# arbobendik/web-ray-tracer

Measured on AMD Instinct MI355X. Metric: Mray/s at 1080p (spp x bounces x pixels / s), higher is better.
Workload: dtype f32

## Files before the change

web-ray-tracer_amd/csrc/flx_frame_common.h:

```cpp
#pragma once
#include "flx_kernels.h"
#include "flx_kernel_util.h"
#include "flx_wavefront_common.h"

namespace flx {

#ifndef FLX_WF_WALK_THREADS
#define FLX_WF_WALK_THREADS 1024
#endif
#ifndef FLX_WF_WAVES_PER_EU
#define FLX_WF_WAVES_PER_EU 4
#endif
#ifndef FLX_WF_LDS_TOTAL
#define FLX_WF_LDS_TOTAL (156 * 1024)
#endif
#ifndef FLX_WF_INNER
#define FLX_WF_INNER 8
#endif
#ifndef FLX_WF_UNROLL
#define FLX_WF_UNROLL 8
#endif
#ifndef FLX_WF_BATCH
#define FLX_WF_BATCH 24
#endif
#ifndef FLX_WF_DRAWS_PER_WAVE
#define FLX_WF_DRAWS_PER_WAVE 16
#endif
#ifndef FLX_FRAME_SHADERS_FRONT
#define FLX_FRAME_SHADERS_FRONT 3
#endif
#ifndef FLX_FRAME_PROLOGUE_WAVES
#define FLX_FRAME_PROLOGUE_WAVES 2
#endif
#ifndef FLX_FRAME_READY_UNITS
#define FLX_FRAME_READY_UNITS 32
#endif

typedef const __attribute__((address_space(4))) FrameArgs *FrameArgsP;
FLX_DEV const FrameArgs &frame_args(FrameArgsP p) { asm volatile("" : "+s"(p)); return *(const FrameArgs *)p; }
FLX_DEV FrameArgsP kernel_frame_args() { return (FrameArgsP)__builtin_amdgcn_kernarg_segment_ptr(); }
#define FLX_ARGS_OF(ab) const FrameArgs &A_ = frame_args(ab); const DeviceScene &sc = A_.sc; const DeviceFrame &fr = A_.fr; const WavefrontBuffers &wb = A_.wb; (void)sc; (void)fr; (void)wb

template <bool VER>
FLX_DEV uint32_t scene_version_of(const DeviceFrame &fr, uint32_t frameIdx) { return VER ? blockIdx.x * fr.frames + frameIdx : 0u; }

template <bool COUNT, bool LV = false, bool VER = false>
FLX_DEV bool shade0_tile(FrameArgsP ab, uint32_t tile, uint32_t lane, float4 h, WorkCounters &cnt, const FrameView *lv = nullptr) {
  uint32_t S, frameIdx, lightBase = 0;
  int tri;
  bool alive, compact;
  f3 camera;
  SurfaceCtx sf;
  float ndcX = 0.0f, ndcY = 0.0f;
  Hit hit;
  {
  FLX_ARGS_OF(ab);
  S = (uint32_t)fr.samples;
  uint32_t px, k;
  tile8_pixel(fr, tile, lane, px, k);
  const bool inFrame = px < fr.width && k < fr.rows;
  frameIdx = inFrame ? frame_index(fr, k) : 0u;
  camera = view_camera(view_at<LV>(fr, lv, frameIdx));
  tri = inFrame ? __float_as_int(h.w) : -1;
  alive = tri != -1 && fr.max_reflections > 0 && length(F3(1.0f, 1.0f, 1.0f) * F3(1.0f, 1.0f, 1.0f)) >= fr.min_importancy * SQRT3;
  hit.suv = F3(h.x, h.y, h.z); hit.triangleId = tri; hit.transformId = 0;
  compact = wb.rec0 != nullptr;
  if (alive) {
    hit.transformId = (int)sc.geometry[3 * tri + 2].y << 1;
    if (VER) { const uint32_t ver = scene_version_of<VER>(fr, frameIdx); hit.transformId += (int)(ver * 2u * sc.n_transforms); lightBase = ver * 6u * sc.n_lights; }
    const uint32_t py_gl = fr.height - 1u - image_row(fr, k);
    float viewDepthPerS;
    Ray pr;
    pr.origin = camera;
    pr.dir = primary_dir_v(fr, view_at<LV>(fr, lv, frameIdx), px, py_gl, ndcX, ndcY, viewDepthPerS);
    const WorkCounters before = cnt;
    shadeSurface<COUNT>(sc, fr, hit, pr, camera, sf, cnt);
    if (COUNT) {
      cnt.shades = before.shades + (cnt.shades - before.shades) * S;
      cnt.atlas_texels = before.atlas_texels + (cnt.atlas_texels - before.atlas_texels) * S;
    }
  }
  }
  for (uint32_t s = 0; s < S; s++) {
    FLX_ARGS_OF(ab);
    const uint32_t pathId = ((tile * S + s) << 6) | lane;
    float4 *rec = wb.rec + (size_t)pathId * 8;
    if (!alive) {
      if (tri != -1) finalize_path<LV>(fr, wb, pathId, F3(0.0f, 0.0f, 0.0f), F3(1.0f, 1.0f, 1.0f), F3(1.0f, 1.0f, 1.0f), lv);
      if (compact) wb.rec0[(size_t)pathId * 3] = make_float4(0.f, 0.f, 0.f, __int_as_float(RF_DEAD));
      else rec[0] = make_float4(0.f, 0.f, 0.f, __int_as_float(RF_DEAD));
      continue;
    }
    PathState p;
    PixelState ps;
    ps.firstRayLength = 1.0f; ps.glassFilter = 0.0f; ps.originalRMEx = 0.0f; ps.originalTPOx = 0.0f;
    ps.renderId.x = ps.renderId.y = ps.renderId.z = ps.renderId.w = 0.0f;
    ps.renderOriginalId = ps.renderId;
    ps.ndc_x = ndcX; ps.ndc_y = ndcY;
    ps.seed = view_at<LV>(fr, lv, frameIdx).random_seed;
    ps.lightBase = lightBase;
    ps.originalColor = F3(1.0f, 1.0f, 1.0f);
    p.hit = hit;
    p.lastHitPoint = camera;
    p.dontFilter = true;
    p.importancyFactor = F3(1.0f, 1.0f, 1.0f);
    const float cosSampleN = flx_cos((float)s);
    ShadeOut so;
    shadeSample(sc, fr, sf, ps, p, camera, cosSampleN, 0, so);
    const int flags = (p.dontFilter ? RF_DONT_FILTER : 0) | (so.needShadow ? RF_NEED_SHADOW : 0) | (so.shadowedNoWalk ? RF_SHADOWED_NO_WALK : 0) |
                      (nextBounceRuns(fr, 0, p.importancyFactor, ps.originalColor) ? 0 : RF_NO_CLOSEST);
    if (compact) {
      if (s == 0u) {
// ... 37 lines not shown
    const FrameView &v = view_at<LV>(fr, lv, frameIdx);
    pr.dir = primary_dir_v(fr, v, px, py_gl, nx, ny, viewDepthPerS);
    pr.origin = view_camera(v);
  }
  const uint32_t visitsBefore = cnt.primary_visits;
  const Hit hp = primaryWalkF(sc, inImage, pr, viewDepthPerS, cnt.primary_visits, xfBase);
  if (COUNT && wb.tileCost && wb.tileCostPrimary) {
    const uint32_t nTiles = ((fr.width + 7u) >> 3) * ((fr.rows + 7u) >> 3);
    atomicAdd(wb.tileCost + nTiles + tile, (unsigned long long)(cnt.primary_visits - visitsBefore));
  }
  float4 h = make_float4(hp.suv.x, hp.suv.y, hp.suv.z, __int_as_float(inImage ? hp.triangleId : -1));
  if (inImage) {
    if (COUNT && hp.triangleId != -1) cnt.primary_hits++;
    hits[(size_t)k * fr.width + px] = h;
  }
  return h;
}

template <bool COUNT, bool LV = false, bool VER = false>
FLX_DEV void shade_path(FrameArgsP ab, uint32_t pathId, WorkCounters &cnt, const FrameView *lv = nullptr) {
  FLX_ARGS_OF(ab);
  float4 *rec = wb.rec + (size_t)pathId * 8;
  uint32_t px, k, s;
  item_pixel(fr, pathId, px, k, s);
  const uint32_t frameIdx = frame_index(fr, k);
  const f3 camera = view_camera(view_at<LV>(fr, lv, frameIdx));
  PathState p;
  PixelState ps;
  ps.firstRayLength = 1.0f; ps.glassFilter = 0.0f; ps.originalRMEx = 0.0f; ps.originalTPOx = 0.0f;
  ps.renderId.x = ps.renderId.y = ps.renderId.z = ps.renderId.w = 0.0f;
  ps.renderOriginalId = ps.renderId;
  const float4 q0 = rec[0], q1 = rec[1], q2 = rec[2], q3 = rec[3], q6 = rec[6], q7 = rec[7];
  const int pb = __float_as_int(q3.w) + 1;
  p.ray.origin = F3(q0.x, q0.y, q0.z);
  p.lastHitPoint = p.ray.origin;
  p.ray.dir = F3(q1.x, q1.y, q1.z);
  p.hit.suv = F3(q2.x, q2.y, q2.z);
  p.hit.triangleId = __float_as_int(q2.w);
  p.hit.transformId = (int)sc.geometry[3 * p.hit.triangleId + 2].y << 1;
  if (VER) { const uint32_t ver = scene_version_of<VER>(fr, frameIdx); p.hit.transformId += (int)(ver * 2u * sc.n_transforms); ps.lightBase = ver * 6u * sc.n_lights; }
  p.dontFilter = (__float_as_int(q0.w) & RF_DONT_FILTER) != 0;
  p.importancyFactor = F3(q6.x, q6.y, q6.z);
  ps.originalColor = F3(q7.x, q7.y, q7.z);
  const uint32_t py_gl = fr.height - 1u - image_row(fr, k);
  float viewDepthPerS;
  (void)primary_dir_v(fr, view_at<LV>(fr, lv, frameIdx), px, py_gl, ps.ndc_x, ps.ndc_y, viewDepthPerS);
  ps.seed = view_at<LV>(fr, lv, frameIdx).random_seed;
  const float cosSampleN = flx_cos((float)s);
  ShadeOut so;
  bounceShade<COUNT>(sc, fr, ps, p, camera, cosSampleN, pb, so, cnt);
  const int flags = (p.dontFilter ? RF_DONT_FILTER : 0) | (so.needShadow ? RF_NEED_SHADOW : 0) | (so.shadowedNoWalk ? RF_SHADOWED_NO_WALK : 0) |
                    (nextBounceRuns(fr, pb, p.importancyFactor, ps.originalColor) ? 0 : RF_NO_CLOSEST);
  rec[0] = make_float4(p.ray.origin.x, p.ray.origin.y, p.ray.origin.z, __int_as_float(flags));
  rec[1] = make_float4(p.ray.dir.x, p.ray.dir.y, p.ray.dir.z, so.shadowLen);
  rec[2] = make_float4(so.shadowRay.origin.x, so.shadowRay.origin.y, so.shadowRay.origin.z, so.baseLuminance.x);
  rec[3] = make_float4(so.shadowRay.dir.x, so.shadowRay.dir.y, so.shadowRay.dir.z, __int_as_float(pb));
  rec[4] = make_float4(so.litColor.x, so.litColor.y, so.litColor.z, 0.0f);
  rec[6] = make_float4(p.importancyFactor.x, p.importancyFactor.y, p.importancyFactor.z, 0.0f);
  rec[7] = make_float4(ps.originalColor.x, ps.originalColor.y, ps.originalColor.z, 0.0f);
}

struct WalkLane {
  int st;
  uint32_t pathId; int flags; int pathBounce; float base;
  Ray nextRay, shadowRay; float shadowLen;
  WalkState w; WalkEntry cur;
  uint32_t v0;
};
FLX_DEV void walkLaneInit(WalkLane &L) {
  L.v0 = 0u;
  L.st = P_EMPTY; L.pathId = 0; L.flags = 0; L.pathBounce = 0; L.base = 0.0f;
  L.nextRay.origin = F3(0.f, 0.f, 0.f); L.nextRay.dir = L.nextRay.origin;
  L.shadowRay = L.nextRay; L.shadowLen = 0.0f;
  walkClearResults(L.w);
  L.w.src = L.nextRay; L.w.tR = L.nextRay; L.w.minLen = 0.0f; L.w.i = 0; L.w.cachedTI = 0;
  L.w.mode = 2;
  L.cur.e0 = L.cur.e1 = L.cur.e2 = make_float4(0.f, 0.f, 0.f, 0.f);
}
FLX_DEV const float4 *pix_part(const DeviceFrame &fr, const WavefrontBuffers &wb, uint32_t id) {
  uint32_t tile0, s0;
  item_tile(fr, id, tile0, s0);
  return wb.pix0 + (((size_t)tile0 << 6) | (id & 63u)) * 3;
}
#define FLX_WALK_LANE_FOLD(LV_, fr_, wb_, compactRecs_, L_, lv_, toShade_, ended_, costed_, stamp_)                              \
  do {                                                                                                                           \
    float4 *rec_ = (wb_).rec + (size_t)(L_).pathId * 8;                                                                          \
    const bool compact_ = (compactRecs_) && (L_).pathBounce == 0;                                                                \
    float4 q4_, q5_, q6_, q7_;                                                                                                   \
    const float4 *pp_ = nullptr;                                                                                                 \
    if (compact_) {                                                                                                              \
      pp_ = pix_part(fr_, wb_, (L_).pathId);                                                                                     \
      q4_ = (wb_).rec0[(size_t)(L_).pathId * 3 + 2]; q7_ = pp_[2];                                                               \
      q5_ = make_float4(0.0f, 0.0f, 0.0f, 0.0f); q6_ = make_float4(1.0f, 1.0f, 1.0f, 0.0f);                                      \
    } else {                                                                                                                     \
      q4_ = rec_[4]; q5_ = rec_[5]; q6_ = rec_[6]; q7_ = rec_[7];                                                                \
    }                                                                                                                            \
    const bool shadowed_ = ((L_).flags & RF_SHADOWED_NO_WALK) || (((L_).flags & RF_NEED_SHADOW) && (L_).w.shadowed);            \
    const f3 localColor_ = shadowed_ ? F3((L_).base, (L_).base, (L_).base) : F3(q4_.x, q4_.y, q4_.z);                            \
    const f3 importancy_ = F3(q6_.x, q6_.y, q6_.z), originalColor_ = F3(q7_.x, q7_.y, q7_.z);                                    \
    const f3 finalColor_ = F3(q5_.x, q5_.y, q5_.z) + localColor_ * importancy_;                                                  \
     \
    const float cost_ = (costed_) ? q5_.w + (float)(((stamp_) - ((uint32_t)(L_).flags >> 8)) & 0xffffffu) : 1.0f;      \
    bool cont_ = (L_).w.tri != -1;                                                                                               \
    if (cont_) cont_ = ((L_).pathBounce + 1) < (fr_).max_reflections && length(importancy_ * originalColor_) >= (fr_).min_importancy * SQRT3;      \
    if (cont_) {                                                                                                                 \
      if (compact_) {                                         \
        const float4 a_ = (wb_).rec0[(size_t)(L_).pathId * 3], bq_ = (wb_).rec0[(size_t)(L_).pathId * 3 + 1], p0_ = pp_[0];      \
        rec_[0] = make_float4(p0_.x, p0_.y, p0_.z, a_.w);                                                                        \
        rec_[1] = make_float4(a_.x, a_.y, a_.z, bq_.w);                                                                          \
        rec_[3] = make_float4(bq_.x, bq_.y, bq_.z, __int_as_float(0));                                                           \
        rec_[6] = make_float4(1.0f, 1.0f, 1.0f, 0.0f);                                                                           \
        rec_[7] = make_float4(q7_.x, q7_.y, q7_.z, 0.0f);                                                                        \
      }                                                                                                                          \
      rec_[5] = make_float4(finalColor_.x, finalColor_.y, finalColor_.z, (costed_) ? cost_ : 0.0f);                                                 \
      rec_[2] = make_float4((L_).w.suv.x, (L_).w.suv.y, (L_).w.suv.z, __int_as_float((L_).w.tri));                               \
      toShade_ = true;                                                                                                           \
    } else {                                                                                                                     \
      finalize_path<LV_>(fr_, wb_, (L_).pathId, finalColor_, importancy_, originalColor_, lv_, cost_);                           \
      ended_ = true;                                                                                                             \
    }                                                                                                                            \
    (L_).st = P_EMPTY;                                                                                                           \
  } while (0)

struct WalkRecord { float4 q0, q1, q2, q3; };
FLX_DEV void walkLaneFetchRecord(const DeviceFrame &fr, const WavefrontBuffers &wb, uint32_t id, bool compactFresh, WalkRecord &R) {
  const float4 *rec = wb.rec + (size_t)id * 8;
  if (compactFresh) {
    const float4 *pp = pix_part(fr, wb, id);
    const float4 a = wb.rec0[(size_t)id * 3], bq = wb.rec0[(size_t)id * 3 + 1];
    const float4 p0 = pp[0], p1 = pp[1], p2 = pp[2];
    R.q0 = make_float4(p0.x, p0.y, p0.z, a.w);
    R.q1 = make_float4(a.x, a.y, a.z, bq.w);
    R.q2 = make_float4(p1.x, p1.y, p1.z, p2.w);
    R.q3 = make_float4(bq.x, bq.y, bq.z, __int_as_float(0));
  } else {
    R.q0 = rec[0]; R.q1 = rec[1]; R.q2 = rec[2]; R.q3 = rec[3];
  }
}
template <bool COUNT>
FLX_DEV bool walkLaneInstall(uint32_t id, const WalkRecord &R, WalkLane &L, WorkCounters &cnt, uint32_t stamp = 0u ) {
  const int fl = __float_as_int(R.q0.w);
  if (fl & RF_DEAD) return true;
  L.pathId = id; L.flags = fl | (int)(stamp << 8); L.base = R.q2.w; L.pathBounce = __float_as_int(R.q3.w);
  L.nextRay.origin = F3(R.q0.x, R.q0.y, R.q0.z);
  L.nextRay.dir = F3(R.q1.x, R.q1.y, R.q1.z);
  L.shadowRay.origin = F3(R.q2.x, R.q2.y, R.q2.z);
  L.shadowRay.dir = F3(R.q3.x, R.q3.y, R.q3.z);
  L.shadowLen = R.q1.w;
  walkClearResults(L.w);
  L.w.mode = (fl & RF_NEED_SHADOW) ? 0 : 1;
  if (COUNT) { if (L.w.mode == 0) cnt.shadow_walks++; if (!(fl & RF_NO_CLOSEST)) cnt.closest_walks++; L.v0 = cnt.closest_visits + cnt.shadow_visits; }
  L.st = (L.w.mode == 1 && (fl & RF_NO_CLOSEST)) ? P_DONE : P_SETUP;
  return false;
}
template <bool COUNT>
FLX_DEV bool walkLaneLoad(const DeviceFrame &fr, const WavefrontBuffers &wb, uint32_t id, bool compactFresh, WalkLane &L, WorkCounters &cnt, uint32_t stamp = 0u) {
  WalkRecord R;
  walkLaneFetchRecord(fr, wb, id, compactFresh, R);
  return walkLaneInstall<COUNT>(id, R, L, cnt, stamp);
}
template <bool COUNT>
FLX_DEV void walkLaneSetup(const DeviceScene &sc, uint32_t nTransforms, const float4 *xf, float2 *myRays, const float4 *walkG, const float4 *ldsEntries, uint32_t ldsCount,
                           WalkLane &L, WorkCounters &cnt) {
  const bool shadowMode = L.w.mode == 0;
  const Ray src = shadowMode ? L.shadowRay : L.nextRay;
  walkSetupRays(sc, nTransforms, xf, myRays, src, shadowMode);
  L.w.tR = src; L.w.cachedTI = 0; L.w.minLen = shadowMode ? L.shadowLen : POW32; L.w.i = (int)sc.walk_root;
  reciprocalOfDir(sc, src.dir, src.origin, L.w.inv, L.w.fastDiv);
  L.st = P_WALKING;
  if (walkFetchG<COUNT>(walkG, ldsEntries, ldsCount, myRays, L.w, L.cur, cnt)) L.st = shadowMode ? P_SWITCH : P_DONE;
}
FLX_DEV void walkLaneSwitch(WalkLane &L) {
  if (L.st == P_SWITCH) {
    if (L.flags & RF_NO_CLOSEST) L.st = P_DONE;
    else { L.w.mode = 1; L.st = P_SETUP; }
  }
}
#ifndef FLX_WF_TRI_EARLY_FETCH
#define FLX_WF_TRI_EARLY_FETCH 1
#endif
#if FLX_WF_TRI_EARLY_FETCH && !(FLX_WF_LINK_KIND && FLX_WF_LINK_ISBOX)
#error "FLX_WF_TRI_EARLY_FETCH needs FLX_WF_LINK_KIND and FLX_WF_LINK_ISBOX: neither the arrival nor the trip's control may wait for the loaded entry"
#endif
FLX_DEV float4 walkAnyFloat4() {
  float x, y, z, w;
  asm volatile("" : "=v"(x)); asm volatile("" : "=v"(y)); asm volatile("" : "=v"(z)); asm volatile("" : "=v"(w));
  return make_float4(x, y, z, w);
}
#if FLX_WF_TRI_EARLY_FETCH
#define FLX_WALK_LANE_STEP(COUNT_, THICK_, walkG_, ldsEntries_, ldsCount_, myRays_, L_, cnt_)                                      \
  do {                                                                                                                           \
    WalkEntry nxt_;                                                                                                              \
    nxt_.e0 = walkAnyFloat4(); nxt_.e1 = walkAnyFloat4(); nxt_.e2 = walkAnyFloat4();                                             \
    if ((L_).st == P_WALKING) {                                                                                                  \
      bool ended_ = false;                                                                                                       \
      uint32_t here_ = (uint32_t)(L_).w.i;                                        \
      if (walkIsBoxL((L_).w)) walkBoxP<THICK_>((L_).w, (L_).cur); else (L_).w.i = __float_as_int((L_).cur.e2.y);                 \
      walkFetchIssue(walkG_, ldsEntries_, ldsCount_, (uint32_t)(L_).w.i, nxt_);                                                  \
      asm("" : "+v"(here_));                                                                                                     \
      if (linkKind(here_) != 1u) ended_ = walkTriT((L_).w, (L_).cur);                                                            \
      if (!ended_) ended_ = walkFetchArrive<COUNT_>(myRays_, (L_).w, nxt_, cnt_);                                                \
      if (ended_) (L_).st = ((L_).w.mode == 0) ? P_SWITCH : P_DONE;                                                              \
    }                                                                                                                            \
    (L_).cur = nxt_;                                                                                                             \
  } while (0)
// ... 68 lines not shown
```

web-ray-tracer_amd/csrc/flx_server.hip:

```cpp
#include <cstddef>
#include <cstdio>
#include <mutex>
#include "flx_server.h"
#include "flx_frame_common.h"

namespace flx {

#ifndef FLX_SERVER_RELAY_GROUPS
#define FLX_SERVER_RELAY_GROUPS 16
#endif
#ifndef FLX_SERVER_SHADERS
#define FLX_SERVER_SHADERS FLX_FRAME_SHADERS_FRONT
#endif
#ifndef FLX_SERVER_SHADERS_DEPTH2_MAX_TILES
#define FLX_SERVER_SHADERS_DEPTH2_MAX_TILES 24
#endif
#ifndef FLX_SERVER_SHADERS_DEPTH2
#define FLX_SERVER_SHADERS_DEPTH2 2
#endif
#ifndef FLX_SERVER_SHADE_PRIO
#define FLX_SERVER_SHADE_PRIO 0
#endif
#ifndef FLX_SERVER_PRIO
#define FLX_SERVER_PRIO 1
// ... 349 lines not shown
            if (fq_pop(ring(RK_WALK, slot), rctl(RK_WALK, slot), idle, nIdle, 1u, lane, id) != 0u) {
              if (mineIdle && id != WF_INVALID) newId = id;
              any = flx_ballot(mineIdle && id != WF_INVALID) != 0ull;
              got = true;
              break;
            }
            if (chunkNext == chunkEnd && fq_load(&rctl(RK_SHADE, slot)[2]) < FQ_LIMIT) {
              uint32_t unit = WF_INVALID;
              if (fq_pop(ring(RK_READY, slot), rctl(RK_READY, slot), 1ull, 1u, 1u, lane, unit) != 0u) {
                unit = __builtin_amdgcn_readfirstlane(unit);
                if (unit != WF_INVALID) { chunkNext = unit << 6; chunkEnd = chunkNext + 64u; }
                else if (lane == 0) { FLX_SERVER_ARGS(); atomicSub(&ctl[SC_ALIVE + slot], 64u); __hip_atomic_fetch_or(sa.error, WF_ERR_RING_SLOT, __ATOMIC_RELAXED, __HIP_MEMORY_SCOPE_SYSTEM); }
              }
            }
            if (chunkNext != chunkEnd && slotOf(chunkNext) == slot) {
              const uint32_t avail = chunkEnd - chunkNext;
              const uint32_t take = nIdle < avail ? nIdle : avail;
              if (mineIdle && rk < take) { newId = chunkNext + rk; newFresh = true; }
              chunkNext += take;
              got = true; any = true;
              break;
            }
          }
          if (!got || !any) break;
        }
        if (newId != WF_INVALID) { FLX_ARGS_OF(ab); walkLaneFetchRecord(fr, wb, newId, newFresh, newRec); }
      }
      if (flx_ballot(L.st == P_DONE) != 0ull) {
        FLX_ARGS_OF(ab);
        const bool compactRecs = wb.rec0 != nullptr;
        bool toShade = false, ended = false;
        const uint32_t slot = slotOf(L.pathId);
        if (L.st == P_DONE) FLX_WALK_LANE_FOLD(true, fr, wb, compactRecs, L, lv, toShade, ended, false, 0u);
        if (flx_ballot(ended) != 0ull) __builtin_amdgcn_fence(__ATOMIC_RELEASE, "workgroup");
        for (uint32_t s = 0; s < depth; s++) {
          fq_push(ring(RK_SHADE, s), rctl(RK_SHADE, s), toShade && slot == s, L.pathId, lane);
          const uint32_t e = (uint32_t)__popcll(flx_ballot(ended && slot == s));
          if (e != 0u && lane == 0) atomicSub(&ctl[SC_ALIVE + s], e);
        }
        worked();
      }
      {
        bool dead = false;
        if (newId != WF_INVALID) dead = walkLaneInstall<false>(newId, newRec, L, cnt);
        if (flx_ballot(dead) != 0ull) {
          const uint32_t dslot = slotOf(newId);
          for (uint32_t sl = 0; sl < depth; sl++) {
            const uint32_t nDead = (uint32_t)__popcll(flx_ballot(dead && dslot == sl));
            if (nDead != 0u && lane == 0) atomicSub(&ctl[SC_ALIVE + sl], nDead);
          }
        }
      }
      if (FLX_SERVER_PRIO) {
        const bool tail = fq_load(&ctl[SC_TILEDRY + P]) != 0u;
        if (tail && flx_ballot(L.st != P_EMPTY && slotOf(L.pathId) == P) != 0ull) __builtin_amdgcn_s_setprio(3); else __builtin_amdgcn_s_setprio(0);
      }
      walkLaneSwitch(L);
      if (flx_ballot(L.st == P_SETUP) != 0ull) {
        FLX_ARGS_OF(ab);
        if (L.st == P_SETUP) walkLaneSetup<false>(sc, nTransforms, VER ? ldsXf + (size_t)slotOf(L.pathId) * nTransforms * 4u : ldsXf, myRays, walkGV, ldsEntriesV, ldsCount, L, cnt);
      }
      if (flx_ballot(L.st == P_WALKING) == 0ull) {
        if (flx_ballot(L.st != P_EMPTY) != 0ull) continue;
        if (fq_load(&ctl[SC_EXIT]) != 0u) break;
        tryRotate();
        if (!mayRefill) __builtin_amdgcn_s_sleep(8);
        continue;
      }
    }
    {
#pragma unroll FLX_WF_UNROLL
      for (int it = 0; it < FLX_WF_INNER; it++) FLX_WALK_LANE_STEP(false, THICK, walkGV, ldsEntriesV, ldsCount, myRays, L, cnt);
    }
  }
  statAdd(SVS_WALK_TRIPS, statTrips); statAdd(SVS_WALK_LANE_TRIPS, statLaneTrips);
  leave();
}

bool server_kernel_fits(const DeviceScene &sc, uint32_t &ldsCount, uint32_t &ldsBytes, uint32_t xfSlots, uint32_t shadeWaves) {
  const uint32_t T = sc.n_transforms;
  if (shadeWaves == 0u) shadeWaves = (uint32_t)FLX_SERVER_SHADERS;
  const uint32_t walkThreads = FLX_WF_WALK_THREADS - 64u * shadeWaves;
  const uint32_t fixed = walkThreads * T * 40u + xfSlots * T * 64u + (SC_WORDS + SC_VIEW_WORDS) * 4u;
  if (fixed + 4096u > (uint32_t)FLX_WF_LDS_TOTAL) return false;
  ldsCount = ((uint32_t)FLX_WF_LDS_TOTAL - fixed) / 48u;
  if (ldsCount > sc.walk_hot) ldsCount = sc.walk_hot;
  ldsBytes = ldsCount * 48u + fixed;
  return true;
}

size_t server_rings_per_group() { return (size_t)SV_RINGS * FQ_SIZE; }

int launch_server(const DeviceScene &sc, const DeviceFrame &fr, const WavefrontBuffers &wb, const ServerArgs &sa, uint32_t compute_units, hipStream_t stream,
                  WalkLdsLaunch *ran) {
  uint32_t ldsCount = 0, ldsBytes = 0;
  const bool ver = sa.blobWords != 0u;
  if (sa.depth < 2u || sa.depth > SV_MAX_DEPTH) return -1;
  const uint32_t shadeWaves = sa.depth == 2u && sa.tilesPerSlot / compute_units <= (uint32_t)FLX_SERVER_SHADERS_DEPTH2_MAX_TILES ? (uint32_t)FLX_SERVER_SHADERS_DEPTH2 : (uint32_t)FLX_SERVER_SHADERS;
  if (!server_kernel_fits(sc, ldsCount, ldsBytes, ver ? sa.depth : 1u, shadeWaves)) return -1;
  if (ver && (sa.blobWords > SV_BLOB_WORDS || sa.blobWords != server_blob_words(sc.n_transforms, sc.n_lights))) return -1;
  static std::once_flag once[64];
  static bool ok[64];
  int dev = 0;
  if (hipGetDevice(&dev) != hipSuccess || dev < 0 || dev >= 64) return -1;
  static const void *const kernels[2][2] = { { (const void *)k_wf_server<false, false>, (const void *)k_wf_server<false, true> },
                                             { (const void *)k_wf_server<true, false>, (const void *)k_wf_server<true, true> } };
  std::call_once(once[dev], [&]() {
    ok[dev] = true;
    for (int k = 0; k < 4; k++) ok[dev] = hipFuncSetAttribute(kernels[k >> 1][k & 1], hipFuncAttributeMaxDynamicSharedMemorySize, 160 * 1024) == hipSuccess && ok[dev];
  });
  if (!ok[dev]) return -1;
  ServerKernelArgs ka;
  ka.fa.sc = sc; ka.fa.fr = fr; ka.fa.wb = wb; ka.sa = sa;
  const uint32_t tilesPerGroup = sa.tilesPerSlot / compute_units;
  uint32_t readyUnits = tilesPerGroup >= 48u ? (uint32_t)FLX_FRAME_READY_UNITS : tilesPerGroup / 2u;
  readyUnits = readyUnits < (uint32_t)FLX_FRAME_READY_UNITS / 4u ? (uint32_t)FLX_FRAME_READY_UNITS / 4u : (readyUnits > (uint32_t)FLX_FRAME_READY_UNITS ? (uint32_t)FLX_FRAME_READY_UNITS : readyUnits);
  uint32_t ldsCountArg = ldsCount, nTransformsArg = sc.n_transforms, shadeWavesArg = shadeWaves;
  void *args[] = { &ka, &ldsCountArg, &nTransformsArg, &shadeWavesArg, &readyUnits };
  (void)hipLaunchKernel(kernels[ver ? 1 : 0][sc.walk_thick_boxes != 0u ? 1 : 0], dim3(compute_units), dim3(FLX_WF_WALK_THREADS), args, ldsBytes, stream);
  if (ran) { ran->ldsCount = ldsCount; ran->pre = 1u; ran->kind = 4u; ran->nTransforms = sc.n_transforms; ran->boxTest = sc.walk_thick_boxes != 0u ? 1 : 0; }
  return 0;
}

}
```

web-ray-tracer_amd/csrc/flx_wavefront.hip:

```cpp
#include <atomic>
#include <mutex>
#include <cstdio>
#include "flx_kernels.h"
#include "flx_kernel_util.h"
#include "flx_wavefront_common.h"
#include "flx_frame_common.h"

namespace flx {


#ifndef FLX_WF_WALK_THREADS
#define FLX_WF_WALK_THREADS 1024
#endif
#ifndef FLX_WF_DRAWS_PER_WAVE
#define FLX_WF_DRAWS_PER_WAVE 16
#endif
#ifndef FLX_WF_PRETRANSFORM
#define FLX_WF_PRETRANSFORM 1
#endif
#ifndef FLX_WF_LDS_TOTAL
#define FLX_WF_LDS_TOTAL (156 * 1024)
#endif
#ifndef FLX_WF_INNER
#define FLX_WF_INNER 8
// ... 568 lines not shown
            }
          }
        }
        chunkNext += take;
      }
      if (COUNT) { const long long tl = clock64(); tLoad += tl - t1; }
      if (st == P_SWITCH) {
        if (flags & RF_NO_CLOSEST) st = P_DONE;
        else { w.mode = 1; st = P_SETUP; }
      }
      if (flx_ballot(st == P_SETUP) != 0ull) {
        if (st == P_SETUP) {
          const bool shadowMode = w.mode == 0;
          const Ray src = shadowMode ? shadowRay : nextRay;
          walkSetupRays(sc, nTransforms, ldsXf, myRays, src, shadowMode);
          w.tR = src; w.cachedTI = 0; w.minLen = shadowMode ? shadowLen : POW32; w.i = (int)sc.walk_root;
          reciprocalOfDir(sc, src.dir, src.origin, w.inv, w.fastDiv);
          st = P_WALKING;
          if (walkFetchP<COUNT>(sc, ldsEntries, ldsCount, myRays, w, cur, cnt)) st = shadowMode ? P_SWITCH : P_DONE;
        }
      }
      if (COUNT) tRefill += clock64() - t1;
      if (flx_ballot(st == P_WALKING) == 0ull) {
        if (itemsLeft || chunkNext != chunkEnd || flx_ballot(st == P_SWITCH || st == P_DONE) != 0ull) continue;
#if FLX_WF_CONSOLIDATE
        if (tailSynced) continue;
#endif
        break;
      }
    }
    long long t2 = COUNT ? clock64() : 0;
#pragma unroll FLX_WF_UNROLL
    for (int it = 0; it < FLX_WF_INNER; it++) {
      if (COUNT) diagIters++;
      if (st == P_WALKING) {
        bool ended = false;
        if (walkIsBoxT(cur)) walkBoxP(w, cur); else ended = walkTriT(w, cur);
        if (!ended) ended = walkFetchP<COUNT>(sc, ldsEntries, ldsCount, myRays, w, cur, cnt);
        if (ended) st = (w.mode == 0) ? P_SWITCH : P_DONE;
      }
#if FLX_DIAG_PAD_SALU
      { uint32_t a = 1, b = 2, c = 3, d = 4;
        for (int k = 0; k < FLX_DIAG_PAD_SALU / 4; k++) asm volatile("s_mov_b32 %0, %1\n s_mov_b32 %1, %2\n s_mov_b32 %2, %3\n s_mov_b32 %3, %0" : "+s"(a), "+s"(b), "+s"(c), "+s"(d) : : "scc"); }
#endif
#if FLX_DIAG_PAD_VALU
      { uint32_t a = lane, b = lane, c = lane, d = lane;
        for (int k = 0; k < FLX_DIAG_PAD_VALU / 4; k++) asm volatile("v_add_u32 %0, %0, 1\n v_add_u32 %1, %1, 1\n v_add_u32 %2, %2, 1\n v_add_u32 %3, %3, 1" : "+v"(a), "+v"(b), "+v"(c), "+v"(d)); }
#endif
    }
    if (COUNT) tInner += clock64() - t2;
  }
#if FLX_WF_CONSOLIDATE
  if (lane == 0) { atomicSub(&tailCtl[TC_LIVE], 1u); if (tailMode) { atomicSub(&tailCtl[TC_TAIL], 1u); atomicAnd(&tailCtl[TC_MASK], ~(1u << (threadIdx.x >> 6))); } }
#endif
  if (outValid) {
    for (uint32_t t = outUsed + lane; t < WF_OUT_CHUNK; t += 64u) listOut[outBase + t] = WF_INVALID;
  }
  if (COUNT && b == 0 && (cnt.closest_visits | cnt.shadow_visits) != 0u) atomicAdd(wb.counters + 23, (unsigned long long)cnt.closest_visits + cnt.shadow_visits);
  flush_counters<COUNT>(cnt, wb.counters);
  if (COUNT && lane == 0) {
    atomicAdd(wb.counters + 8 + 2 * (b < 4 ? b : 3), (unsigned long long)diagIters); atomicAdd(wb.counters + 9 + 2 * (b < 4 ? b : 3), (unsigned long long)diagBatches);
    const unsigned long long life = (unsigned long long)(clock64() - tStart);
    if (b == 0) {
      atomicAdd(wb.counters + 16, (unsigned long long)tFold); atomicAdd(wb.counters + 17, (unsigned long long)tRefill);
      atomicAdd(wb.counters + 18, (unsigned long long)tInner); atomicAdd(wb.counters + 19, life); atomicAdd(wb.counters + 20, 1ull);
      atomicAdd(wb.counters + 21, (unsigned long long)tLoad); atomicAdd(wb.counters + 22, (unsigned long long)tTail);
    }
    if (b < 4) {
      atomicAdd(wb.counters + 24 + 3 * b, life); atomicAdd(wb.counters + 25 + 3 * b, 1ull); atomicMax(wb.counters + 26 + 3 * b, life);
    }
  }
}

#ifndef FLX_FRAME_WALK_PRIO
#define FLX_FRAME_WALK_PRIO 0
#endif
#ifndef FLX_FRAME_SHADE_PRIO
#define FLX_FRAME_SHADE_PRIO 0
#endif
#ifndef FLX_FRAME_SHADERS
#define FLX_FRAME_SHADERS 2
#endif
#ifndef FLX_FRAME_SHADERS_FRONT
#define FLX_FRAME_SHADERS_FRONT 3
#endif
#ifndef FLX_FRAME_PROLOGUE_WAVES
#define FLX_FRAME_PROLOGUE_WAVES 2
#endif
#ifndef FLX_FRAME_GROUPS_PER_CU
#define FLX_FRAME_GROUPS_PER_CU 1
#endif
#ifndef FLX_FRAME_AUTO_MAX_ITEMS
#define FLX_FRAME_AUTO_MAX_ITEMS (64u << 20)
#endif
#ifndef FLX_FRAME_AUTO_MAX_ITEMS_FRONT
#define FLX_FRAME_AUTO_MAX_ITEMS_FRONT (128u << 20)
#endif
template <bool COUNT, bool FRONT, bool STAMP, bool THICK>
__device__ __forceinline__ void wf_frame_body(uint32_t total_items, uint32_t ldsCount, uint32_t nTransforms, uint32_t shadeWaves, uint32_t readyUnits) {
  const uint32_t n = total_items;
  if (n == 0u) return;
  const FrameArgsP argBase = kernel_frame_args();
#define FLX_FRAME_ARGS() FLX_ARGS_OF(argBase)
  const uint32_t WALK_WAVES = FLX_WF_WALK_THREADS / 64u - shadeWaves;
  uint32_t *frameRings; uint32_t samples; bool compactRecs;
  { FLX_FRAME_ARGS(); frameRings = wb.frameRings; samples = (uint32_t)fr.samples; compactRecs = wb.rec0 != nullptr; }
  extern __shared__ float4 ldsAll[];
  float4 *ldsEntries = ldsAll;
  float4 *ldsXf = ldsAll + (size_t)ldsCount * 3u;
  uint32_t *ctl = (uint32_t *)(ldsXf + (size_t)nTransforms * 4u);
  uint32_t *shadeRing = frameRings + (size_t)blockIdx.x * WF_FRAME_RINGS * FQ_SIZE, *walkRing = shadeRing + FQ_SIZE, *readyRing = walkRing + FQ_SIZE;
  constexpr bool front = FRONT;
  const uint32_t perTile = samples * 64u;
  float2 *raysBase = (float2 *)(ctl + FC_WORDS);
  {
    FLX_FRAME_ARGS();
    for (uint32_t t = threadIdx.x; t < ldsCount * 3u; t += FLX_WF_WALK_THREADS) ldsEntries[t] = sc.walk[t];
    for (uint32_t t = threadIdx.x; t < nTransforms * 4u; t += FLX_WF_WALK_THREADS) {
      const uint32_t tr = t >> 2, k = t & 3u, iI = 2u * tr + 1u;
      ldsXf[t] = k < 3u ? sc.rotation[3u * iI + k] : sc.shift[iI];
    }
  }
  if (threadIdx.x < (uint32_t)FC_WORDS) ctl[threadIdx.x] = 0u;
  __syncthreads();
  const uint32_t lane = threadIdx.x & 63u;
  const uint32_t wave = threadIdx.x >> 6;
  WorkCounters cnt = {};

  const uint32_t nTiles = n / perTile;
  auto makeTile = [&]() -> uint32_t {
    if (!FRONT) return 2u;
    FLX_FRAME_ARGS();
    uint32_t take = 0, tile = 0;
    if (lane == 0 && fq_load(&ctl[FC_RQ + 2]) < readyUnits) {
      const uint32_t before = atomicAdd(&ctl[FC_ALIVE], perTile);
      if (before + perTile > FQ_ALIVE_MAX) atomicSub(&ctl[FC_ALIVE], perTile);
      else { tile = atomicAdd(wb.walkQueue, 1u); take = 1; }
    }
    take = __builtin_amdgcn_readfirstlane(take);
    tile = __builtin_amdgcn_readfirstlane(tile);
    if (take == 0u) return 0u;
    if (tile >= nTiles) {
      if (lane == 0) atomicSub(&ctl[FC_ALIVE], perTile);
      return 2u;
    }
    if (wb.tileOrder) tile = __builtin_amdgcn_readfirstlane(wb.tileOrder[tile]);
    tile += wb.item_base / perTile;
    const float4 h = primary_tile<COUNT>(argBase, tile, lane, cnt);
    const bool runs = shade0_tile<COUNT>(argBase, tile, lane, h, cnt);
    if (flx_ballot(runs) == 0ull) {
      if (lane == 0) atomicSub(&ctl[FC_ALIVE], perTile);
    } else {
      for (uint32_t s0 = 0; s0 < samples; s0 += 64u)
        fq_push(readyRing, ctl + FC_RQ, s0 + lane < samples, tile * samples + s0 + lane, lane);
    }
    return 1u;
  };

  if (wave >= WALK_WAVES) {
    uint32_t idle = 0;
    bool frontDone = !front;
    uint32_t inject; { FLX_FRAME_ARGS(); inject = wb.inject; } asm volatile("" : "+s"(inject));
    if (FLX_FRAME_SHADE_PRIO) __builtin_amdgcn_s_setprio(FLX_FRAME_SHADE_PRIO);
    const long long tStartShade = COUNT ? clock64() : 0;
    uint32_t thinMarks = 0;
    for (;;) {
      FLX_FRAME_ARGS();
// ... 215 lines not shown
      }
      const long long tB2 = COUNT ? clock64() : 0; if (COUNT) tRefillT += tB2 - tB1;
      walkLaneSwitch(L);
      if (flx_ballot(L.st == P_SETUP) != 0ull) {
        FLX_FRAME_ARGS();
        if (L.st == P_SETUP) walkLaneSetup<COUNT>(sc, nTransforms, ldsXf, myRays, FLX_FETCH_G, FLX_FETCH_L, ldsCount, L, cnt);
      }
      if (COUNT) { const long long tB3 = clock64(); tSetupT += tB3 - tB2; tBlock += tB3 - tB0; }
      if (flx_ballot(L.st == P_WALKING) == 0ull) {
        if (flx_ballot(L.st != P_EMPTY) != 0ull) continue;
        if (front) {
          if (fq_load(&ctl[FC_DRY]) != 0u && chunkNext == chunkEnd && fq_load(&ctl[FC_ALIVE]) == 0u) break;
        } else if (!itemsLeft && chunkNext == chunkEnd && fq_load(&ctl[FC_ALIVE]) == 0u) break;
        if (fq_load(&ctl[FC_WQ + 2]) == 0u && (front ? (fq_load(&ctl[FC_RQ + 2]) == 0u || fq_load(&ctl[FC_SQ + 2]) >= FQ_LIMIT)
                                                     : !(itemsLeft && fq_load(&ctl[FC_SQ + 2]) < FQ_LIMIT && fq_load(&ctl[FC_ALIVE]) + 256u <= FQ_ALIVE_MAX))) {
          FLX_FRAME_ARGS();
          if (++idleSpins > (wb.watchdog ? wb.watchdog : FQ_WATCHDOG)) {
            if (lane == 0 && wb.error) __hip_atomic_fetch_or(wb.error, WF_ERR_WALK_WATCHDOG, __ATOMIC_RELAXED, __HIP_MEMORY_SCOPE_SYSTEM);
            if (COUNT && lane == 0) { for (uint32_t k = 0; k < 8u; k++) atomicMax(wb.counters + 50 + k, (unsigned long long)fq_load(&ctl[k]) + 1ull); atomicAdd(wb.counters + 58, 1ull); }
            break;
          }
          __builtin_amdgcn_s_sleep(8);
        }
        continue;
      }
    }
    const long long tT0 = COUNT ? clock64() : 0;
    {
#pragma unroll FLX_WF_UNROLL
      for (int it = 0; it < FLX_WF_INNER; it++) FLX_WALK_LANE_STEP(COUNT, THICK, FLX_FETCH_G, FLX_FETCH_L, ldsCount, myRays, L, cnt);
    }
    if (COUNT) tTrips += clock64() - tT0;
  }
  FLX_FRAME_ARGS();
  if (COUNT && (cnt.closest_visits | cnt.shadow_visits) != 0u) atomicAdd(wb.counters + 23, (unsigned long long)cnt.closest_visits + cnt.shadow_visits);
#if FLX_BOX_FALLBACK_COUNT
  if (COUNT && wave < WALK_WAVES) atomicAdd(wb.counters + 59, (unsigned long long)L.w.boxTests | (unsigned long long)L.w.boxExact << 32);
#endif
  if (COUNT && lane == 0) {
    const unsigned long long life = (unsigned long long)(clock64() - tStart);
    atomicAdd(wb.counters + 64, life); atomicMax(wb.counters + 65, life); atomicAdd(wb.counters + 66, 1ull);
    atomicAdd(wb.counters + 67, (unsigned long long)tBlock); atomicAdd(wb.counters + 68, (unsigned long long)tFoldT); atomicAdd(wb.counters + 69, (unsigned long long)tRefillT); atomicAdd(wb.counters + 70, (unsigned long long)tSetupT);
    atomicAdd(wb.counters + 71, (unsigned long long)tTrips); atomicAdd(wb.counters + 72, nBlocks); atomicAdd(wb.counters + 73, nOuter);
    atomicAdd(wb.counters + 74, (unsigned long long)tAcqT); atomicAdd(wb.counters + 75, (unsigned long long)tFoldOnlyT);
  }
  flush_counters<COUNT>(cnt, wb.counters);
#undef FLX_FETCH_G
#undef FLX_FETCH_L
#undef FLX_FRAME_ARGS
}
template <bool COUNT, bool FRONT>
__global__ __launch_bounds__(FLX_WF_WALK_THREADS, FLX_WF_WAVES_PER_EU) void k_wf_frame(FrameArgs , uint32_t total_items,
                                                                                    uint32_t ldsCount, uint32_t nTransforms, uint32_t shadeWaves, uint32_t readyUnits) {
  wf_frame_body<COUNT, FRONT, !FRONT, true>(total_items, ldsCount, nTransforms, shadeWaves, readyUnits);
}
template <bool COUNT, bool FRONT>
__global__ __launch_bounds__(FLX_WF_WALK_THREADS, FLX_WF_WAVES_PER_EU) void k_wf_frame_flat(FrameArgs , uint32_t total_items,
                                                                                         uint32_t ldsCount, uint32_t nTransforms, uint32_t shadeWaves, uint32_t readyUnits) {
  wf_frame_body<COUNT, FRONT, !FRONT, false>(total_items, ldsCount, nTransforms, shadeWaves, readyUnits);
}
template <bool COUNT>
__global__ __launch_bounds__(FLX_WF_WALK_THREADS, FLX_WF_WAVES_PER_EU) void k_wf_frame_stamped(FrameArgs , uint32_t total_items,
                                                                                            uint32_t ldsCount, uint32_t nTransforms, uint32_t shadeWaves, uint32_t readyUnits) {
  wf_frame_body<COUNT, true, true, true>(total_items, ldsCount, nTransforms, shadeWaves, readyUnits);
}
template <bool COUNT>
__global__ __launch_bounds__(FLX_WF_WALK_THREADS, FLX_WF_WAVES_PER_EU) void k_wf_frame_stamped_flat(FrameArgs , uint32_t total_items,
                                                                                                 uint32_t ldsCount, uint32_t nTransforms, uint32_t shadeWaves, uint32_t readyUnits) {
  wf_frame_body<COUNT, true, true, false>(total_items, ldsCount, nTransforms, shadeWaves, readyUnits);
}
static const void *frame_kernel(int which, bool count, bool thick) {
  static const void *const kernels[3][2][2] = {
    { { (const void *)k_wf_frame_flat<false, false>, (const void *)k_wf_frame<false, false> }, { (const void *)k_wf_frame_flat<true, false>, (const void *)k_wf_frame<true, false> } },
    { { (const void *)k_wf_frame_flat<false, true>, (const void *)k_wf_frame<false, true> }, { (const void *)k_wf_frame_flat<true, true>, (const void *)k_wf_frame<true, true> } },
    { { (const void *)k_wf_frame_stamped_flat<false>, (const void *)k_wf_frame_stamped<false> }, { (const void *)k_wf_frame_stamped_flat<true>, (const void *)k_wf_frame_stamped<true> } } };
  return kernels[which][count ? 1 : 0][thick ? 1 : 0];
}

static bool frame_kernel_fits(const DeviceScene &sc, bool withFront, uint32_t &ldsCount, uint32_t &ldsBytes) {
  const uint32_t T = sc.n_transforms;
  const uint32_t walkThreads = FLX_WF_WALK_THREADS - 64u * (withFront ? (uint32_t)FLX_FRAME_SHADERS_FRONT : (uint32_t)FLX_FRAME_SHADERS);
  const uint32_t fixed = walkThreads * T * 40u + T * 64u + FC_WORDS * 4u;
  if (!FLX_WF_PRETRANSFORM || fixed + 4096u > (uint32_t)FLX_WF_LDS_TOTAL) return false;
  ldsCount = ((uint32_t)FLX_WF_LDS_TOTAL - fixed) / 48u;
  if (ldsCount > sc.walk_hot) ldsCount = sc.walk_hot;
  ldsBytes = ldsCount * 48u + fixed;
  return true;
}

template <typename SetAttributes>
static bool dynamic_lds_ready(int family, SetAttributes set) {
  static std::once_flag once[2][64];
  static bool ok[2][64];
  int dev = 0;
  if (hipGetDevice(&dev) != hipSuccess || dev < 0 || dev >= 64) return false;
  std::call_once(once[family][dev], [&]() { ok[family][dev] = set(); });
  return ok[family][dev];
}
static bool set_lds_limit(const void *kernel) { return hipFuncSetAttribute(kernel, hipFuncAttributeMaxDynamicSharedMemorySize, 160 * 1024) == hipSuccess; }

static bool frame_kernel_wanted(const DeviceScene &sc, const DeviceFrame &fr, uint32_t item_count, int organisation, bool withFront, uint32_t &ldsCountF, uint32_t &ldsBytesF) {
  const bool wanted = organisation == 2 || (organisation == 0 && item_count <= (withFront ? (uint32_t)FLX_FRAME_AUTO_MAX_ITEMS_FRONT : (uint32_t)FLX_FRAME_AUTO_MAX_ITEMS));
  return wanted && fr.max_reflections >= 1 && frame_kernel_fits(sc, withFront, ldsCountF, ldsBytesF);
}
bool wavefront_front_in_kernel(const DeviceScene &sc, const DeviceFrame &fr, uint32_t item_count, int organisation) {
  uint32_t a = 0, b = 0;
  return frame_kernel_wanted(sc, fr, item_count, organisation, true, a, b) && (uint32_t)fr.samples * 64u * 2u <= FQ_ALIVE_MAX;
}

int launch_wavefront(const DeviceScene &sc, const DeviceFrame &fr, const WavefrontBuffers &wbIn, uint32_t compute_units, bool count,
                     int organisation, hipEvent_t walk0_begin, hipEvent_t walk0_end, hipStream_t stream, WalkLdsLaunch *ran) {
  WavefrontBuffers wb = wbIn;
  const bool fused = wb.front == 2u;
  if (fused) wb.front = 0u;
  {
    uint32_t ldsCountF = 0, ldsBytesF = 0;
    if (wb.frameRings != nullptr && frame_kernel_wanted(sc, fr, wb.item_count, organisation, wb.front != 0u, ldsCountF, ldsBytesF) &&
        dynamic_lds_ready(0, []() {
          bool ok = true;
          for (int k = 0; k < 12; k++) ok = set_lds_limit(frame_kernel(k >> 2, (k & 1) != 0, (k & 2) != 0)) && ok;
          return ok;
        })) {
      const uint32_t total = wb.item_count;
      const uint32_t pixels = total / (uint32_t)(fr.samples > 0 ? fr.samples : 1);
      const uint32_t shadeBlocks = (pixels + 255u) / 256u;
      FrameArgs fa; fa.sc = sc; fa.fr = fr; fa.wb = wb;
      if (wb.front) {  }
      else if (fused) { if (count) hipLaunchKernelGGL(k_wf_front<true>, dim3(shadeBlocks), dim3(256), 0, stream, fa, total); else hipLaunchKernelGGL(k_wf_front<false>, dim3(shadeBlocks), dim3(256), 0, stream, fa, total); }
      else if (count) hipLaunchKernelGGL(k_wf_shade0<true>, dim3(shadeBlocks), dim3(256), 0, stream, fa, total);
      else hipLaunchKernelGGL(k_wf_shade0<false>, dim3(shadeBlocks), dim3(256), 0, stream, fa, total);
      if (walk0_begin) (void)hipEventRecord(walk0_begin, stream);
      const uint32_t shadeWaves = wb.front ? (uint32_t)FLX_FRAME_SHADERS_FRONT : (uint32_t)FLX_FRAME_SHADERS;
      const dim3 grid(compute_units * (uint32_t)FLX_FRAME_GROUPS_PER_CU), block(FLX_WF_WALK_THREADS);
      const uint32_t tilesPerGroup = (total / ((uint32_t)fr.samples * 64u)) / compute_units;
#ifndef FLX_FRAME_READY_DIV
#define FLX_FRAME_READY_DIV 2u
#endif
      uint32_t readyUnits = tilesPerGroup >= 48u ? (uint32_t)FLX_FRAME_READY_UNITS : tilesPerGroup / FLX_FRAME_READY_DIV;
      readyUnits = readyUnits < (uint32_t)FLX_FRAME_READY_UNITS / 4u ? (uint32_t)FLX_FRAME_READY_UNITS / 4u : (readyUnits > (uint32_t)FLX_FRAME_READY_UNITS ? (uint32_t)FLX_FRAME_READY_UNITS : readyUnits);
      uint32_t totalArg = total, ldsCountArg = ldsCountF, nTransformsArg = sc.n_transforms, shadeWavesArg = shadeWaves;
      void *args[] = { &fa, &totalArg, &ldsCountArg, &nTransformsArg, &shadeWavesArg, &readyUnits };
      (void)hipLaunchKernel(frame_kernel(wb.front ? (wb.stampCosts ? 2 : 1) : 0, count, sc.walk_thick_boxes != 0u), grid, block, args, ldsBytesF, stream);
      if (walk0_end) (void)hipEventRecord(walk0_end, stream);
      if (ran) { ran->ldsCount = ldsCountF; ran->pre = 1u; ran->kind = wb.front ? 3u : 2u; ran->nTransforms = sc.n_transforms; ran->boxTest = sc.walk_thick_boxes != 0u ? 1 : 0; }
      return wb.front ? 3 : 2;
    }
  }
  if (wb.front) return -1;
  const uint32_t total = wb.item_count;
  const uint32_t maxBlocks = compute_units * 8u;
  const uint32_t T = sc.n_transforms;
  const uint32_t rayBytes = FLX_WF_WALK_THREADS * T * 40u + T * 64u + 128u;
  const bool pre = FLX_WF_PRETRANSFORM && rayBytes <= 148u * 1024u && rayBytes <= (uint32_t)FLX_WF_LDS_TOTAL;
  const uint32_t ldsBudget = (uint32_t)FLX_WF_LDS_TOTAL - (pre ? rayBytes : 0u);
  uint32_t ldsCount = ldsBudget / 48u;
  if (ldsCount > sc.walk_hot) ldsCount = sc.walk_hot;
  const uint32_t ldsBytes = ldsCount * 48u + (pre ? rayBytes : 0u);
  uint32_t perCu = (160u * 1024u) / (ldsBytes > 20480u ? ldsBytes : 20480u);
  if (perCu > 8u) perCu = 8u;
  const uint32_t walkBlocks = compute_units * perCu;
  if (!dynamic_lds_ready(1, []() {
        int ok = 1;
        for (const void *k : { (const void *)k_wf_walk<true>, (const void *)k_wf_walk<false>, (const void *)k_wf_walk_pre<true, true>, (const void *)k_wf_walk_pre<false, true>,
                               (const void *)k_wf_walk_pre<true, false>, (const void *)k_wf_walk_pre<false, false> }) ok &= (int)set_lds_limit(k);
        return ok != 0;
      })) return -2;
// ... 40 lines not shown
```

web-ray-tracer_amd/csrc/flx_wavefront_common.h:

```cpp
#pragma once
#include "flx_kernels.h"
#include "flx_kernel_util.h"

namespace flx {

constexpr uint32_t WF_INVALID = 0xffffffffu;
constexpr uint32_t WF_IN_CHUNK = 256;
constexpr uint32_t WF_OUT_CHUNK = 256;

enum { P_EMPTY = 0, P_WALKING = 1, P_DONE = 2, P_SWITCH = 3, P_SETUP = 4 };

constexpr int RF_DEAD = 1, RF_DONT_FILTER = 2, RF_NEED_SHADOW = 4, RF_SHADOWED_NO_WALK = 8;
constexpr int RF_NO_CLOSEST = 16;


template <bool LV = false>
__device__ __forceinline__ void finalize_path(const DeviceFrame &fr, const WavefrontBuffers &wb, uint32_t pathId, f3 finalColor,
                                              f3 importancy, f3 originalColor, const FrameView *lv = nullptr, float cost = 1.0f ) {
  uint32_t px, k, s;
  item_pixel(fr, pathId, px, k, s);
  const size_t P = (size_t)fr.rows * fr.width;
  const size_t o = (size_t)k * fr.width + px;
  const f3 r = finalColor + importancy * view_ambient(view_at<LV>(fr, lv, frame_index(fr, k)));
  wb.sampleRadiance[(size_t)s * P + o] = make_float4(r.x, r.y, r.z, cost);
  if (s == (uint32_t)fr.samples - 1u) wb.lastOriginal[o] = make_float4(originalColor.x, originalColor.y, originalColor.z, 1.0f);
}


}
```

Baseline: 12450.

## Split walk-lane fold into early fetch, rebuild compact records from lane state

Splits the walk-lane fold macro into a fetch step and a compute/write step so the record loads can be issued earlier. On the compact first-bounce path it builds rec[0..3] from the lane's nextRay/shadowRay registers instead of re-reading rec0 and pix0 from global memory. It also raises the front shader waves from 3 to 4 and adds a cap on transform count that turns off the fused frame kernel when a scene has more than 4 transforms. Together these trim global loads in the fold but change the walk/shade wave split, and the new cap can force large-transform scenes onto the fallback path.

```diff
diff --git a/web-ray-tracer_amd/csrc/flx_frame_common.h b/web-ray-tracer_amd/csrc/flx_frame_common.h
--- a/web-ray-tracer_amd/csrc/flx_frame_common.h
+++ b/web-ray-tracer_amd/csrc/flx_frame_common.h
@@ -27,7 +27,10 @@
 #define FLX_WF_DRAWS_PER_WAVE 16
 #endif
 #ifndef FLX_FRAME_SHADERS_FRONT
-#define FLX_FRAME_SHADERS_FRONT 3
+#define FLX_FRAME_SHADERS_FRONT 4
+#endif
+#ifndef FLX_WF_MAX_TRANSFORMS
+#define FLX_WF_MAX_TRANSFORMS 4
 #endif
 #ifndef FLX_FRAME_PROLOGUE_WAVES
 #define FLX_FRAME_PROLOGUE_WAVES 2
@@ -231,6 +234,60 @@
   item_tile(fr, id, tile0, s0);
   return wb.pix0 + (((size_t)tile0 << 6) | (id & 63u)) * 3;
 }
+#ifndef FLX_WF_FOLD_EARLY
+#define FLX_WF_FOLD_EARLY 1
+#endif
+#if FLX_WF_FOLD_EARLY
+struct WalkFold { float4 q4, q5, q6, q7; bool compact; };
+#define FLX_WALK_LANE_FOLD_FETCH(fr_, wb_, compactRecs_, L_, F_)                                                                 \
+  do {                                                                                                                           \
+    const float4 *a4_ = (wb_).rec + (size_t)(L_).pathId * 8 + 4, *a7_ = a4_ + 3;                                                 \
+    (F_).compact = (compactRecs_) && (L_).pathBounce == 0;                                                                       \
+    if ((F_).compact) { a4_ = (wb_).rec0 + (size_t)(L_).pathId * 3 + 2; a7_ = pix_part(fr_, wb_, (L_).pathId) + 2; }             \
+     \
+    (F_).q4 = *a4_; (F_).q7 = *a7_;                                                                                              \
+    if (!(F_).compact) { (F_).q5 = a4_[1]; (F_).q6 = a4_[2]; }       \
+  } while (0)
+#define FLX_WALK_LANE_FOLD_WITH(LV_, fr_, wb_, compactRecs_, L_, F_, lv_, toShade_, ended_, costed_, stamp_)                     \
+  do {                                                                                                                           \
+    float4 *rec_ = (wb_).rec + (size_t)(L_).pathId * 8;                                                                          \
+    const bool compact_ = (F_).compact;                                                                                          \
+    const float4 q4_ = (F_).q4, q7_ = (F_).q7;                                                                                   \
+    float4 q5_ = make_float4(0.0f, 0.0f, 0.0f, 0.0f), q6_ = make_float4(1.0f, 1.0f, 1.0f, 0.0f);                                 \
+    if (!compact_) { q5_ = (F_).q5; q6_ = (F_).q6; }                                                                             \
+    const bool shadowed_ = ((L_).flags & RF_SHADOWED_NO_WALK) || (((L_).flags & RF_NEED_SHADOW) && (L_).w.shadowed);            \
+    const f3 localColor_ = shadowed_ ? F3((L_).base, (L_).base, (L_).base) : F3(q4_.x, q4_.y, q4_.z);                            \
+    const f3 importancy_ = F3(q6_.x, q6_.y, q6_.z), originalColor_ = F3(q7_.x, q7_.y, q7_.z);                                    \
+    const f3 finalColor_ = F3(q5_.x, q5_.y, q5_.z) + localColor_ * importancy_;                                                  \
+     \
+    const float cost_ = (costed_) ? q5_.w + (float)(((stamp_) - ((uint32_t)(L_).flags >> 8)) & 0xffffffu) : 1.0f;      \
+    bool cont_ = (L_).w.tri != -1;                                                                                               \
+    if (cont_) cont_ = ((L_).pathBounce + 1) < (fr_).max_reflections && length(importancy_ * originalColor_) >= (fr_).min_importancy * SQRT3;      \
+    if (cont_) {                                                                                                                 \
+      if (compact_) {                                         \
+                                                                            \
+        rec_[0] = make_float4((L_).nextRay.origin.x, (L_).nextRay.origin.y, (L_).nextRay.origin.z, __int_as_float((L_).flags & 0xff));             \
+        rec_[1] = make_float4((L_).nextRay.dir.x, (L_).nextRay.dir.y, (L_).nextRay.dir.z, (L_).shadowLen);                                         \
+        rec_[3] = make_float4((L_).shadowRay.dir.x, (L_).shadowRay.dir.y, (L_).shadowRay.dir.z, __int_as_float(0));                                \
+        rec_[6] = make_float4(1.0f, 1.0f, 1.0f, 0.0f);                                                                           \
+        rec_[7] = make_float4(q7_.x, q7_.y, q7_.z, 0.0f);                                                                        \
+      }                                                                                                                          \
+      rec_[5] = make_float4(finalColor_.x, finalColor_.y, finalColor_.z, (costed_) ? cost_ : 0.0f);                                                 \
+      rec_[2] = make_float4((L_).w.suv.x, (L_).w.suv.y, (L_).w.suv.z, __int_as_float((L_).w.tri));                               \
+      toShade_ = true;                                                                                                           \
+    } else {                                                                                                                     \
+      finalize_path<LV_>(fr_, wb_, (L_).pathId, finalColor_, importancy_, originalColor_, lv_, cost_);                           \
+      ended_ = true;                                                                                                             \
+    }                                                                                                                            \
+    (L_).st = P_EMPTY;                                                                                                           \
+  } while (0)
+#define FLX_WALK_LANE_FOLD(LV_, fr_, wb_, compactRecs_, L_, lv_, toShade_, ended_, costed_, stamp_)                              \
+  do {                                                                                                                           \
+    WalkFold fold_;                                                                                                              \
+    FLX_WALK_LANE_FOLD_FETCH(fr_, wb_, compactRecs_, L_, fold_);                                                                 \
+    FLX_WALK_LANE_FOLD_WITH(LV_, fr_, wb_, compactRecs_, L_, fold_, lv_, toShade_, ended_, costed_, stamp_);                     \
+  } while (0)
+#else
 #define FLX_WALK_LANE_FOLD(LV_, fr_, wb_, compactRecs_, L_, lv_, toShade_, ended_, costed_, stamp_)                              \
   do {                                                                                                                           \
     float4 *rec_ = (wb_).rec + (size_t)(L_).pathId * 8;                                                                          \
@@ -248,12 +305,11 @@
     const f3 localColor_ = shadowed_ ? F3((L_).base, (L_).base, (L_).base) : F3(q4_.x, q4_.y, q4_.z);                            \
     const f3 importancy_ = F3(q6_.x, q6_.y, q6_.z), originalColor_ = F3(q7_.x, q7_.y, q7_.z);                                    \
     const f3 finalColor_ = F3(q5_.x, q5_.y, q5_.z) + localColor_ * importancy_;                                                  \
-     \
-    const float cost_ = (costed_) ? q5_.w + (float)(((stamp_) - ((uint32_t)(L_).flags >> 8)) & 0xffffffu) : 1.0f;      \
+    const float cost_ = (costed_) ? q5_.w + (float)(((stamp_) - ((uint32_t)(L_).flags >> 8)) & 0xffffffu) : 1.0f;               \
     bool cont_ = (L_).w.tri != -1;                                                                                               \
     if (cont_) cont_ = ((L_).pathBounce + 1) < (fr_).max_reflections && length(importancy_ * originalColor_) >= (fr_).min_importancy * SQRT3;      \
     if (cont_) {                                                                                                                 \
-      if (compact_) {                                         \
+      if (compact_) {                                                                                                            \
         const float4 a_ = (wb_).rec0[(size_t)(L_).pathId * 3], bq_ = (wb_).rec0[(size_t)(L_).pathId * 3 + 1], p0_ = pp_[0];      \
         rec_[0] = make_float4(p0_.x, p0_.y, p0_.z, a_.w);                                                                        \
         rec_[1] = make_float4(a_.x, a_.y, a_.z, bq_.w);                                                                          \
@@ -261,7 +317,7 @@
         rec_[6] = make_float4(1.0f, 1.0f, 1.0f, 0.0f);                                                                           \
         rec_[7] = make_float4(q7_.x, q7_.y, q7_.z, 0.0f);                                                                        \
       }                                                                                                                          \
-      rec_[5] = make_float4(finalColor_.x, finalColor_.y, finalColor_.z, (costed_) ? cost_ : 0.0f);                                                 \
+      rec_[5] = make_float4(finalColor_.x, finalColor_.y, finalColor_.z, (costed_) ? cost_ : 0.0f);                              \
       rec_[2] = make_float4((L_).w.suv.x, (L_).w.suv.y, (L_).w.suv.z, __int_as_float((L_).w.tri));                               \
       toShade_ = true;                                                                                                           \
     } else {                                                                                                                     \
@@ -270,6 +326,7 @@
     }                                                                                                                            \
     (L_).st = P_EMPTY;                                                                                                           \
   } while (0)
+#endif
 
 struct WalkRecord { float4 q0, q1, q2, q3; };
 FLX_DEV void walkLaneFetchRecord(const DeviceFrame &fr, const WavefrontBuffers &wb, uint32_t id, bool compactFresh, WalkRecord &R) {
diff --git a/web-ray-tracer_amd/csrc/flx_server.hip b/web-ray-tracer_amd/csrc/flx_server.hip
--- a/web-ray-tracer_amd/csrc/flx_server.hip
+++ b/web-ray-tracer_amd/csrc/flx_server.hip
@@ -455,7 +455,7 @@
   if (shadeWaves == 0u) shadeWaves = (uint32_t)FLX_SERVER_SHADERS;
   const uint32_t walkThreads = FLX_WF_WALK_THREADS - 64u * shadeWaves;
   const uint32_t fixed = walkThreads * T * 40u + xfSlots * T * 64u + (SC_WORDS + SC_VIEW_WORDS) * 4u;
-  if (fixed + 4096u > (uint32_t)FLX_WF_LDS_TOTAL) return false;
+  if (fixed + 4096u > (uint32_t)FLX_WF_LDS_TOTAL || T > (uint32_t)FLX_WF_MAX_TRANSFORMS) return false;
   ldsCount = ((uint32_t)FLX_WF_LDS_TOTAL - fixed) / 48u;
   if (ldsCount > sc.walk_hot) ldsCount = sc.walk_hot;
   ldsBytes = ldsCount * 48u + fixed;
diff --git a/web-ray-tracer_amd/csrc/flx_wavefront.hip b/web-ray-tracer_amd/csrc/flx_wavefront.hip
--- a/web-ray-tracer_amd/csrc/flx_wavefront.hip
+++ b/web-ray-tracer_amd/csrc/flx_wavefront.hip
@@ -674,7 +674,7 @@
 #define FLX_FRAME_SHADERS 2
 #endif
 #ifndef FLX_FRAME_SHADERS_FRONT
-#define FLX_FRAME_SHADERS_FRONT 3
+#define FLX_FRAME_SHADERS_FRONT 4
 #endif
 #ifndef FLX_FRAME_PROLOGUE_WAVES
 #define FLX_FRAME_PROLOGUE_WAVES 2
@@ -1056,6 +1056,7 @@
   const uint32_t walkThreads = FLX_WF_WALK_THREADS - 64u * (withFront ? (uint32_t)FLX_FRAME_SHADERS_FRONT : (uint32_t)FLX_FRAME_SHADERS);
   const uint32_t fixed = walkThreads * T * 40u + T * 64u + FC_WORDS * 4u;
   if (!FLX_WF_PRETRANSFORM || fixed + 4096u > (uint32_t)FLX_WF_LDS_TOTAL) return false;
+  if (T > (uint32_t)FLX_WF_MAX_TRANSFORMS) return false;
   ldsCount = ((uint32_t)FLX_WF_LDS_TOTAL - fixed) / 48u;
   if (ldsCount > sc.walk_hot) ldsCount = sc.walk_hot;
   ldsBytes = ldsCount * 48u + fixed;
diff --git a/web-ray-tracer_amd/csrc/flx_wavefront_common.h b/web-ray-tracer_amd/csrc/flx_wavefront_common.h
--- a/web-ray-tracer_amd/csrc/flx_wavefront_common.h
+++ b/web-ray-tracer_amd/csrc/flx_wavefront_common.h
@@ -12,6 +12,7 @@
 
 constexpr int RF_DEAD = 1, RF_DONT_FILTER = 2, RF_NEED_SHADOW = 4, RF_SHADOWED_NO_WALK = 8;
 constexpr int RF_NO_CLOSEST = 16;
+static_assert((RF_DEAD | RF_DONT_FILTER | RF_NEED_SHADOW | RF_SHADOWED_NO_WALK | RF_NO_CLOSEST) < (1 << 8), "the record flags must fit below bit 8");
 
 
 template <bool LV = false>
```

After: 13040 (median of 6 runs). +4.7%, better.
